# riveSunder/therldaisyworld

Hardware: AMD Instinct MI355X
Metric: cell-updates/sec (grid x batch), fused stencil+growth step (higher is better)
Workload: dtype f32

## Files before the change

### therldaisyworld_amd/csrc/dw_api.hip

```cpp
#include <hip/hip_runtime.h>

#include <cmath>
#include <cstdarg>
#include <cstdio>
#include <cstdlib>
#include <cstring>
#include <memory>
#include <new>
#include <optional>
#include <type_traits>
#include <vector>

#include "../../include/daisyworld_hip.h"
#include "dw_kernels.hpp"
#include "dw_host_util.hpp"
#include "dw_plan.hpp"
#include "dw_series.hpp"
#include "dw_episode_staging.hpp"

using namespace dw;

static thread_local char g_err[512] = "";

static int fail(int code, const char* fmt, ...) {
// ... 23 lines not shown
static thread_local int t_fail_in = 0;
struct DeviceMem {
    static int alloc(void** p, size_t n) {
        if (t_fail_in > 0 && --t_fail_in == 0) return hipErrorOutOfMemory;
        return hipMalloc(p, n);
    }
    static int release(void* p) { return hipFree(p); }
};
struct PinnedMem {
    static int alloc(void** p, size_t n) { return hipHostMalloc(p, n, hipHostMallocDefault); }
    static int release(void* p) { return hipHostFree(p); }
};
template <class T> using DevBuf = Buf<T, DeviceMem>;
template <class T> using PinnedBuf = Buf<T, PinnedMem>;

struct dw_handle {
    dw_params prm;
    hipStream_t stream = nullptr;
    bool own_stream = false;
    size_t cells = 0;
    DevBuf<plane_t> L16[2];
    DevBuf<plane_t> D16[2];
    int cur = 0;
    DevBuf<double> L64;
    DevBuf<double> D64;
    DevBuf<float> U32L;
    DevBuf<float> U32D;
    UnqKind unq_kind = UNQ_F64;
    UnqOwner unq = OWN_NONE;
    bool have_state = false;
    bool stepped = false;
    double L_last = 0.0;
    bool L_per_world = false;
    bool P_per_world = false;
    DevBuf<int> idx;
    DevBuf<double> st;
    DevBuf<int> action;
    DevBuf<int> action_tmp;
    bool have_agents = false;
    DevBuf<StatsDev> stats2[2];
    size_t stats_bytes = 0;
    int sp = 0;
    DevBuf<uint4> fixq;
    unsigned int qcap = 0;
    DevBuf<int> redo_tiles;
    Switches sw{};
// ... 82 lines not shown
        return with_bool(post, [&](auto POST) { return f(L, D, POST); });
    });
}

struct SyncOnExit {
    hipStream_t stream;
    bool armed = true;
    explicit SyncOnExit(hipStream_t s) : stream(s) {}
    ~SyncOnExit() { if (armed) (void)hipStreamSynchronize(stream); }
    void disarm() { armed = false; }
};

static int alloc_failed(int rc, const char* what, size_t bytes) {
    (void)hipGetLastError();
    const hipError_t e = static_cast<hipError_t>(rc);
    return fail(e == hipErrorOutOfMemory ? DW_ENOMEM : DW_EHIP, "allocating %s (%zu bytes) failed: %s", what, bytes,
                hipGetErrorString(e));
}
template <class B>
static int reserve(B& buf, const char* what, size_t need, size_t first_size = 0) {
    const int rc = buf.reserve(need, first_size);
    return rc ? alloc_failed(rc, what, need) : DW_OK;
}

static int alloc_group(dw_handle* h, const char* what, std::initializer_list<GroupItem<DeviceMem>> group) {
    static int fail_left = -1;
    if (h->created && fail_left < 0)
        if (const char* e = test_hook("DW_TEST_FAIL_GROUP_ALLOC")) fail_left = std::atoi(e);
    const bool armed = h->created && fail_left > 0;
    if (armed) t_fail_in = (int)group.size();
    const int rc = dw::alloc_group(group);
    if (armed && t_fail_in == 0) --fail_left;
    t_fail_in = 0;
    size_t bytes = 0;
    for (const auto& g : group) bytes += g.bytes;
    return rc ? alloc_failed(rc, what, bytes) : DW_OK;
}

static void release_unquantised(dw_handle* h) {
    if (h->unq != OWN_NONE || !h->U32L.get()) return;
    for (const auto& sn : h->snap)
        if (sn.valid && sn.unq == OWN_PREV) return;
    if (h->cells * 2 * sizeof(float) < ((size_t)1 << 30)) return;
    (void)hipStreamSynchronize(h->stream);
    h->U32L.reset();
    h->U32D.reset();
}

static void drop_unquantised_previous(dw_handle* h) {
    if (h->unq == OWN_PREV) { h->unq = OWN_NONE; h->stepped = false; }
    release_unquantised(h);
}

static int ensure_u32(dw_handle* h) {
    const size_t n = sizeof(float) * h->cells;
    return alloc_group(h, "two float32 planes", {{h->U32L, n}, {h->U32D, n}});
}

static int ensure_f64(dw_handle* h) {
    const size_t n = sizeof(double) * h->cells;
    return alloc_group(h, "two float64 planes", {{h->L64, n}, {h->D64, n}});
}

static int run_episode_impl(dw_handle* h, int32_t nsteps, const double* L_schedule, int policy_mode,
                            const uint8_t* use_table, const int8_t* table, uint32_t threshold_k,
                            uint8_t* world_alive, uint8_t* agent_ok, dw_world_stats* trace = nullptr,
                            dw_temp_stats* temps = nullptr);
static bool episode_kernel_applies(const dw_handle* h);
enum EpisodeForm { EPISODE_STEPWISE, EPISODE_WORKGROUP, EPISODE_WAVE };
static EpisodeForm episode_form(const dw_handle* h);
static EpisodeForm episode_mlp_form(const dw_handle* h, size_t* lds_bytes = nullptr);
static int worlds_per_block(int cells) { return cells <= 256 ? 4 : (cells <= 1024 ? 2 : 1); }
static int observe_into_scratch(dw_handle* h, double L_init, size_t extra_bytes, bool reward_tail = false);

static int ensure_scratch(dw_handle* h, size_t bytes) { return reserve(h->scratch, "scratch", bytes); }

static int ensure_ep_buf(dw_handle* h, size_t bytes) {
    return reserve(h->ep_buf, "the episode staging buffer", bytes, (size_t)4 << 20);
}

struct EpisodeBuffers {
    using R = EpisodeStaging;
    dw_handle* h;
    const EpisodeStaging S;
    unsigned char* img = nullptr;
    std::vector<PhysF32> p32_own;
    std::vector<unsigned char> ut_own;

    EpisodeBuffers(dw_handle* h_, const EpisodeStaging& S_) : h(h_), S(S_) {}
    bool out_direct = false;
    int alloc(bool staged, bool inputs_only = false) {
        if (int rc = ensure_ep_buf(h, S.total)) return rc;
        if (!staged) return DW_OK;
        const size_t image = inputs_only ? S.off[R::WORLD_ALIVE] : S.total;
        if (int rc = reserve(h->ep_pinned, "the page-locked episode staging", image, (size_t)1 << 20)) return rc;
        img = h->ep_pinned.get();
        out_direct = inputs_only;
        return DW_OK;
    }
    template <class T = unsigned char>
    T* dev(R::Region r) const { return S.at<T>(h->ep_buf.get(), r); }
// ... 549 lines not shown
                           o.zero_me, o.zero_n);
    } else if (exact) {
        const FusedExactArgs A = exact_args();
        with_bool(pstats != nullptr, [&](auto STATS) {
            with_fused_layout(pl, [&](auto MODE, auto PACK) {
                with_bool(pl.sym_albedo, [&](auto SYM) {
                    hipLaunchKernelGGL((step_stream_fused2_exact<MODE, PACK, STATS, SYM>), grid, dim3(256), 0, h->stream, A);
                });
            });
        });
    } else {
        with_bool(pstats != nullptr, [&](auto STATS) {
            with_fused_layout(pl, [&](auto MODE, auto PACK) {
                hipLaunchKernelGGL((step_stream_fused2<MODE, PACK, STATS>), grid, dim3(256), 0, h->stream, inL, inD, o.L, o.D, g,
                                   P1, P2, o.zero_me, o.zero_n, pstats, thr_hi);
            });
        });
    }
    HIPCHK(hipGetLastError());
    step_done(h, L2, false);
    return DW_OK;
}

static int launch_agents(dw_handle* h, const int* d_action, int act_b, int act_n, bool standalone = false,
                         double* d_reward = nullptr, unsigned char* d_done = nullptr, unsigned char* d_ok = nullptr) {
    const dw_params& p = h->prm;
    if (p.n_agents == 0) return DW_OK;
    NEED(h->have_state, DW_ESTATE, "no state uploaded");
    NEED(h->have_agents, DW_ESTATE, "no agents uploaded (call dw_upload_agents or dw_init_random)");
    NEED(p.collision_mode == 0 || standalone, DW_EINVAL,
         "collision_mode=1: call dw_update_agents, apply the collision pass (it consumes the caller's RNG) to the "
         "downloaded agent states, upload them, then dw_step without actions");
    const int blocks = (p.batch + 63) / 64;
    with_planes(h, h->unq == OWN_CUR, h->cur, [&](auto* L, auto* D) {
        using T = elem_t<decltype(L)>;
        hipLaunchKernelGGL(agents_update<T>, dim3(blocks), dim3(64), 0, h->stream, L, D, h->idx.get(), h->st.get(), d_action,
                           act_b, act_n, p.batch, p.n_agents, p.height, p.width, p.agent_gamma,
                           p.collision_mode == 0 ? 1 : 0, d_reward, d_done, d_ok);
    });
    HIPCHK(hipGetLastError());
    return DW_OK;
}

static int stage_host_actions(dw_handle* h, const int32_t* action, int b, int n) {
    const dw_params& p = h->prm;
    NEED(b >= 0 && n >= 0 && b <= p.batch && n <= p.n_agents, DW_EINVAL,
// ... 460 lines not shown
    if (!use_device_actions && nsteps >= 1 && h->have_state && !cur_quantised(h)) {
        int rc = launch_forward(h, L);
        if (rc) return rc;
        advance();
        s0 = 1;
    }
    const bool big_packed = h->plan.allow_fuse && h->plan.packed && h->cells >= ((size_t)1 << 23);
    if (!use_device_actions && nsteps - s0 > 1 && h->have_state && h->prm.height * h->prm.width <= 4096 && !big_packed &&
        (h->prm.n_agents == 0 || h->have_agents) && episode_kernel_applies(h)) {
        std::vector<double> Ls;
        while (s0 < nsteps) {
            const int k = nsteps - s0 < 4096 ? nsteps - s0 : 4096;
            Ls.resize(k);
            for (int i = 0; i < k; ++i) { Ls[i] = L; advance(); }
            int rc = run_episode_impl(h, k, Ls.data(), kPolicySkipAgents, nullptr, nullptr, 5, nullptr, nullptr);
            if (rc) return rc;
            s0 += k;
        }
        *L_io = L;
        return DW_OK;
    }
    if (!use_device_actions && h->plan.allow_fuse && h->have_state && nsteps - s0 >= 3) {
        drop_unquantised_previous(h);
        HIPCHK(hipEventRecord(h->evf0, h->stream));
        int launched = 0;
        while (nsteps - s0 >= 3) {
            const double L1 = L;
            advance();
            const double L2 = L;
            advance();
            int rc = launch_forward_fused2(h, L1, L2);
            if (rc) return rc;
            s0 += 2;
            launched += 1;
        }
        HIPCHK(hipEventRecord(h->evf1, h->stream));
        h->fused_launches = launched;
    }
    for (int s = s0; s < nsteps; ++s) {
        int rc;
        if (use_device_actions) {
            rc = launch_agents(h, h->action.get(), h->prm.batch, h->prm.n_agents);
            if (rc) return rc;
        }
        rc = launch_forward(h, L);
        if (rc) return rc;
        advance();
    }
    *L_io = L;
    return DW_OK;
}

static bool ensemble_pairs(const dw_handle* h) { return h->plan.trace_pairs && h->prm.precision == DW_PRECISION_FAST; }

static int check_per_world(const WorldRows& rows, const dw_world_params* worlds, const double* L_schedule, size_t nsteps, size_t B) {
    for (size_t i = 0; i < nsteps * B; ++i)
        NEED(std::isfinite(L_schedule[i]) && L_schedule[i] >= 0.0, DW_EINVAL,
             "L_schedule[step %zu][world %zu] = %g: a luminosity is finite and not negative", i / B, i % B, L_schedule[i]);
    for (size_t b = 0; worlds && b < B; ++b) {
        if (check_params(&rows.params(b)) != DW_OK) {
// ... 556 lines not shown
    NEED(h->have_state && h->have_agents, DW_ESTATE, "no state / agents");
    const int B = p.batch, N = p.n_agents;
    const size_t K = (size_t)nsteps, bn = (size_t)B * N;
    NEED(bn > 0, DW_EINVAL, "no agents");
    for (int b = 0; b < B; ++b) {
        NEED(!member_a || (member_a[b] >= 0 && member_a[b] < n_members), DW_EINVAL, "world %d: member out of range", b);
        NEED(!member_b || (member_b[b] >= 0 && member_b[b] < n_members), DW_EINVAL, "world %d: member out of range", b);
    }
    NEED(n_members == 1 || (member_a && member_b), DW_EINVAL, "several parameter sets need both member maps");
    NEED_SHARED_L(h, "the episode's first observation");
    const size_t wbytes = sizeof(double) * 1808 * (size_t)n_members;
    EpisodeRegions regions;
    regions.rows = K; regions.mlp = true; regions.trace = records; regions.temps = temps != nullptr;
    const EpisodeStaging S(K, (size_t)B, (size_t)N, regions);
    using R = EpisodeStaging;
    const size_t o_ma = S.off[R::MEMBER_A], o_mb = S.off[R::MEMBER_B], o_p32 = S.off[R::P32], o_ls = S.off[R::LS];
    if (temps)
        if (int rc = alloc_group(h, "the temperature reduction", {{h->temp_part, temp_part_bytes(h)}})) return rc;
    if (int erc = ensure_ep_buf(h, S.total)) return erc;
    if (params) {
        if (h->mlp_members != n_members) {
            h->mlp_w.reset();
            h->mlp_members = 0;
            if (int rc = reserve(h->mlp_w, "the parameter sets", wbytes)) return rc;
            h->mlp_members = n_members;
        }
    }
    const double* d_w = h->mlp_w.get();
    const int* d_ma = member_a ? reinterpret_cast<const int*>(h->ep_buf.get() + o_ma) : nullptr;
    const int* d_mb = member_b ? reinterpret_cast<const int*>(h->ep_buf.get() + o_mb) : nullptr;
    double* d_r = S.at<double>(h->ep_buf.get(), R::REWARD);
    unsigned char* d_d = S.at<unsigned char>(h->ep_buf.get(), R::DONE);
    StatsDev* const d_rows = S.at<StatsDev>(h->ep_buf.get(), R::TRACE);
    TempStatsDev* const d_trows = reinterpret_cast<TempStatsDev*>(h->ep_buf.get() + S.temps_off());
    SyncOnExit guard(h->stream);
    if (params) HIPCHK(hipMemcpyAsync(h->mlp_w.get(), params, wbytes, hipMemcpyHostToDevice, h->stream));
    if (member_a) HIPCHK(hipMemcpyAsync(h->ep_buf.get() + o_ma, member_a, sizeof(int) * B, hipMemcpyHostToDevice, h->stream));
    if (member_b) HIPCHK(hipMemcpyAsync(h->ep_buf.get() + o_mb, member_b, sizeof(int) * B, hipMemcpyHostToDevice, h->stream));
    const int Cc = p.height * p.width;
    const int wpb = worlds_per_block(Cc);
    size_t lds = 0;
    const EpisodeForm form = episode_mlp_form(h, &lds);
    const bool wave_kernel = form == EPISODE_WAVE, small = records ? form == EPISODE_WAVE : form != EPISODE_STEPWISE;
    if (records) lds = episode_mlp_wave_trace_lds_bytes(Cc, N);
    std::vector<PhysF32> p32;
    SyncOnExit guard2(h->stream);
    size_t t = 0;
// ... 734 lines not shown
    if (pl.kind == STEP_STREAM) {
        const StripGeom& g = pl.sgeom;
        snprintf(buf, buflen,
                 "step_stream_%s<halo=%s> wave-strip=%dx256 cells, register window + DPP neighbours, %d-row blocks in "
                 "flight%s, %d strips, grid=%d x 256 threads (4 strips each), XCD-chunked",
                 prec, halo_name[pl.halo], g.SR,
                 p.precision == DW_PRECISION_EXACT ? DW_STREAM_RB_EXACT : DW_STREAM_RB_FAST,
                 p.precision == DW_PRECISION_EXACT ? ", in-wave float64 fix-up from an LDS queue" : "", g.nstrips,
                 g.chunk * 8);
        if (pl.allow_fuse) {
            const size_t n = std::strlen(buf);
            snprintf(buf + n, buflen - n, "; dw_step_n fuses step pairs (step_stream_fused2%s%s",
                     p.precision == DW_PRECISION_EXACT ? "_exact" : "",
                     pl.seam_strips ? "_seam_pw, format buffer accesses" : (pl.fmt_planes ? "_fmt_pw, format buffer accesses" : ""));
            if (pl.seam_strips) {
                const size_t m = std::strlen(buf);
                snprintf(buf + m, buflen - m, ", seam strips: %d x %d columns + %d columns of %d row bands per wave", pl.seam_geom.ncs,
                         kSeamCols, pl.left_geom.cols_per_strip, pl.left_geom.wpr);
            }
            if (pl.row_landing) {
                const size_t m = std::strlen(buf);
                snprintf(buf + m, buflen - m, ", rows land in place: step_stream_fused2_land_seam_pw + _land_left_pw");
            }
            const size_t m = std::strlen(buf);
            snprintf(buf + m, buflen - m, ")");
        }
    } else if (pl.kind == STEP_TILED) {
        const int TR = (256 / pl.tcq) * pl.rpt;
        snprintf(buf, buflen,
                 "step_tiled<TCQ=%d,RPT=%d,%s> tile=%dx%d cells, %zu B LDS/workgroup, %d tiles, grid=%d x 256 threads, "
                 "XCD-chunked",
                 pl.tcq, pl.rpt, prec, TR, pl.tcq * 4, pl.tile_lds, pl.geom.ntiles, pl.geom.chunk * 8);
    } else {
        snprintf(buf, buflen, "step_generic<%s> one thread per cell, grid=(%d,%d) x 256 threads", prec,
                 (p.height * p.width + 255) / 256, p.batch);
    }
    {
        const size_t n = std::strlen(buf);
        snprintf(buf + n, buflen - n, pl.trace_pairs ? "; trace: step pairs" : "; trace: single steps");
    }
    {
        const size_t n = std::strlen(buf);
        snprintf(buf + n, buflen - n, pl.pw_stream ? "; per-world L: wave strips" : "; per-world L: generic");
    }
    {
        static const char* const form_name[] = {"launches per step", "workgroup (LDS)", "one wave per world"};
// ... 84 lines not shown
```

### therldaisyworld_amd/csrc/dw_plan.hpp

```cpp
#pragma once
#include <climits>
#include <cmath>
#include <cstddef>
#include <cstdio>
#include <cstdlib>
#include <cstring>

#include "../../include/daisyworld_hip.h"
#include "dw_types.hpp"

namespace dw {

struct Switches {
    bool no_sym = false, no_pack = false, no_fuse = false, no_ring = false, no_fmt_planes = false, no_seam_strips = false,
         no_row_landing = false,
         no_episode_kernel = false,
         no_episode_wave = false, no_agent_fuse = false, no_agent_preapply = false, first_f64 = false,
         first_generic = false, force_rescan = false, test_hooks = false;
    int pack_min_strips = -1, strip_rows = 0, tile_rpt = 0, queue_cap = -1, mismatch_cap = -1, trace_rows = 0, frame_ring = 0;
    double first_slack = -1.0;
    char kernel[16] = {0};
    char text[256] = {0};
};
inline const char* test_hook(const char* name) {
    return std::getenv("DW_TEST_HOOKS") ? std::getenv(name) : nullptr;
}
inline Switches read_switches() {
    Switches w;
    auto note = [&](const char* name, const char* val) {
        const size_t n = std::strlen(w.text);
        snprintf(w.text + n, sizeof(w.text) - n, "%s%s%s%s", n ? " " : "", name, val ? "=" : "", val ? val : "");
    };
    auto flag = [&](const char* name, bool& dst) { if (std::getenv(name)) { dst = true; note(name, nullptr); } };
    auto num = [&](const char* name, int& dst, bool test) {
        if (const char* e = test ? test_hook(name) : std::getenv(name)) { dst = std::atoi(e); note(name, e); }
    };
    w.test_hooks = std::getenv("DW_TEST_HOOKS") != nullptr;
    flag("DW_NO_SYM", w.no_sym); flag("DW_NO_PACK", w.no_pack); flag("DW_NO_FUSE", w.no_fuse); flag("DW_NO_RING", w.no_ring);
    flag("DW_NO_FMT_PLANES", w.no_fmt_planes); flag("DW_NO_SEAM_STRIPS", w.no_seam_strips);
    flag("DW_NO_ROW_LANDING", w.no_row_landing);
    flag("DW_NO_EPISODE_KERNEL", w.no_episode_kernel); flag("DW_NO_EPISODE_WAVE", w.no_episode_wave);
    flag("DW_NO_AGENT_FUSE", w.no_agent_fuse); flag("DW_NO_AGENT_PREAPPLY", w.no_agent_preapply);
    flag("DW_FIRST_STEP_F64", w.first_f64); flag("DW_FIRST_GENERIC", w.first_generic);
    num("DW_PACK_MIN_STRIPS", w.pack_min_strips, false); num("DW_STRIP_ROWS", w.strip_rows, false);
    num("DW_TILE_RPT", w.tile_rpt, false);
    num("DW_TEST_QUEUE_CAP", w.queue_cap, true); num("DW_TEST_MISMATCH_CAP", w.mismatch_cap, true);
    num("DW_TEST_TRACE_ROWS", w.trace_rows, true);
    num("DW_TEST_FRAME_RING", w.frame_ring, true);
    if (test_hook("DW_TEST_FORCE_RESCAN")) { w.force_rescan = true; note("DW_TEST_FORCE_RESCAN", nullptr); }
    if (const char* e = test_hook("DW_TEST_FIRST_SLACK")) { w.first_slack = std::atof(e); note("DW_TEST_FIRST_SLACK", e); }
    if (const char* e = std::getenv("DW_KERNEL")) { snprintf(w.kernel, sizeof(w.kernel), "%s", e); note("DW_KERNEL", e); }
    return w;
}

inline dw_params with_world_params(dw_params p, const dw_world_params& w) {
    p.p = w.p; p.g = w.g; p.S = w.S; p.sigma = w.sigma; p.gamma = w.gamma; p.q = w.q; p.q2 = w.q2; p.dt = w.dt;
    p.albedo_bare = w.albedo_bare; p.albedo_light = w.albedo_light; p.albedo_dark = w.albedo_dark;
    p.temp_optimal = w.temp_optimal;
    return p;
}
inline dw_world_params world_params_of(const dw_params& p) {
    return dw_world_params{p.p, p.g, p.S, p.sigma, p.gamma, p.q, p.q2, p.dt, p.albedo_bare, p.albedo_light, p.albedo_dark,
                           p.temp_optimal};
}
inline bool albedo_symmetric(double bare, double light, double dark) { return (dark - bare) == -(light - bare); }
inline bool worlds_symmetric(const dw_world_params* worlds, size_t B) {
    for (size_t b = 0; b < B; ++b)
        if (!albedo_symmetric(worlds[b].albedo_bare, worlds[b].albedo_light, worlds[b].albedo_dark)) return false;
    return true;
}

// ... 167 lines not shown
enum StepKind { STEP_GENERIC, STEP_TILED, STEP_STREAM };
struct StepPlan {
    StepKind kind = STEP_GENERIC;
    int halo = 0;
    bool packed = false;
    bool allow_fuse = false;
    int fused_mode = kFusedOvl;
    bool fmt_planes = false;
    bool seam_strips = false;
    FusedGeom seam_geom{}, left_geom{};
    bool row_landing = false;
    bool trace_pairs = false;
    bool sym_albedo = false;
    int tcq = 0, rpt = 0;
    Geom geom{};
    size_t tile_lds = 0;
    StripGeom sgeom{};
    FusedGeom fgeom{};
    int first_prec = 2;
    bool first_stream = false;
    FirstGeom first_geom{};
    bool need_fixq = false;
    bool pw_stream = false;
};

inline int halo_form(int W) { return W < 256 ? 3 : (W == 256 ? 0 : (W % 256 == 0 ? 1 : 2)); }

inline int strip_rows(long groups, int H, long target) {
    int sr = 64;
    while (sr > 8 && groups * ((H + sr - 1) / sr) < target) sr >>= 1;
    return H < sr ? H : sr;
}

inline int strip_rows_or_override(const Switches& sw, int cap, long groups, int H, long target) {
    if (sw.strip_rows < 1) return strip_rows(groups, H, target);
    const int want = sw.strip_rows < cap ? sw.strip_rows : cap;
    return H < want ? H : want;
}

inline long seam_waves_per_world(int W, int nrs) {
    const int n_full = W / kSeamCols, L = W - kSeamCols * n_full;
    const int G = L ? 64 / (L / 4 + 2) : 1;
    return (long)nrs * n_full + (L ? (nrs + G - 1) / G : 0);
}
inline bool seam_layout(const FusedGeom& f, FusedGeom* seam, FusedGeom* left) {
    const int n_full = f.W / kSeamCols, L = f.W - kSeamCols * n_full;
// ... 44 lines not shown
        if (sw.mismatch_cap >= 0 && sw.mismatch_cap < kMismatchCap) mcap = sw.mismatch_cap;
        g.force_rescan = sw.force_rescan ? 1 : 0;
        s.allow_fuse = !sw.no_fuse;
        const bool ring = p.width == 1024 && !sw.no_ring;
        s.fused_mode = p.width <= 256 ? kFusedRot : (ring ? kFusedRing : kFusedOvl);
        FusedGeom& f = s.fgeom;
        f.B = p.batch; f.H = p.height; f.W = p.width;
        f.SR = g.SR;
        f.nrs = g.nrs;
        f.lpw = g.lpw; f.wpr = g.wpr;
        f.cols_per_strip = p.width <= 256 ? 256 : (ring ? 1024 : 248);
        f.ncs = s.packed ? 1 : (p.width + f.cols_per_strip - 1) / f.cols_per_strip;
        f.nstrips = (int)(groups * f.nrs * f.ncs);
        f.nwg = ring ? f.nstrips : (f.nstrips + 3) / 4;
        f.chunk = (f.nwg + 7) / 8;
        f.qcap = g.qcap;
        f.mcap = mcap;
        f.sure_need = 9 * p.n_agents + 9 * mcap + 1;
        s.trace_pairs = s.allow_fuse && !s.packed && s.fused_mode != kFusedRing;
        s.fmt_planes = p.precision == DW_PRECISION_FAST && s.allow_fuse && !s.packed && s.fused_mode == kFusedOvl && !sw.no_fmt_planes &&
                       (size_t)p.height * p.width * sizeof(plane_t) < ((size_t)1 << 31);
        s.seam_strips = s.fmt_planes && !sw.no_seam_strips && seam_layout(f, &s.seam_geom, &s.left_geom);
        s.row_landing = s.seam_strips && !sw.no_row_landing;
    } else if (quads && p.width >= 64) {
        s.kind = STEP_TILED;
        const int Wq = p.width / 4;
        if (Wq >= 64) {
            s.tcq = 64; s.rpt = 4;
            if (sw.tile_rpt == 2 || sw.tile_rpt == 4 || sw.tile_rpt == 8) s.rpt = sw.tile_rpt;
        }
        else if (Wq >= 32) { s.tcq = 32; s.rpt = 4; }
        else { s.tcq = 16; s.rpt = 2; }
        const int TR = (256 / s.tcq) * s.rpt;
        Geom& g = s.geom;
        g.B = p.batch; g.H = p.height; g.W = p.width; g.Wq = Wq;
        g.tiles_r = (p.height + TR - 1) / TR;
        g.tiles_c = (Wq + s.tcq - 1) / s.tcq;
        g.ntiles = p.batch * g.tiles_r * g.tiles_c;
        g.chunk = (g.ntiles + 7) / 8;
        g.qcap = kMaxFix;
        if (sw.queue_cap >= 0 && sw.queue_cap < kMaxFix) g.qcap = sw.queue_cap;
        s.tile_lds = (size_t)2 * (TR + 2) * (s.tcq + 2) * 4 * sizeof(float);
    }
    s.need_fixq = p.precision == DW_PRECISION_EXACT && s.kind == STEP_TILED;
    s.pw_stream = s.kind == STEP_STREAM && !s.packed;
    s.first_prec = p.precision == DW_PRECISION_FAST ? 1 : (p.precision == DW_PRECISION_EXACT && !sw.first_f64 ? 3 : 2);
// ... 17 lines not shown
```

### therldaisyworld_amd/csrc/dw_step_fused.hpp

```cpp
#pragma once
#include <type_traits>
#include "dw_step_stream.hpp"
#include "dw_types.hpp"

namespace dw {


template <typename TI>
__device__ inline unsigned int exact1_word(const TI* __restrict__ pL, const TI* __restrict__ pD, int H, int W,
                                           int r, int c, const PhysF64& Pa) {
    const int rr = wrap_near2(r, H), cc = wrap_near2(c, W);
    const int ru = rr == 0 ? H - 1 : rr - 1, rd = rr == H - 1 ? 0 : rr + 1;
    const int cl = cc == 0 ? W - 1 : cc - 1, cr = cc == W - 1 ? 0 : cc + 1;
    const int rows[3] = {ru, rr, rd}, cols[3] = {cl, cc, cr};
    unsigned int w1[9];
#pragma unroll
    for (int x = 0; x < 3; ++x)
#pragma unroll
        for (int y = 0; y < 3; ++y) {
            const size_t o = (size_t)rows[x] * W + cols[y];
            w1[x * 3 + y] = (unsigned)(float)pL[o] | ((unsigned)(float)pD[o] << 16);
        }
    const NewCoverF64 s1 = cell_f64_lean(Pa, w1);
    return (unsigned)dw_round3_k(s1.nl) | ((unsigned)dw_round3_k(s1.nd) << 16);
// ... 10 lines not shown
            int rr = r + a - 1, cc = c + e - 1;
            rr = rr < 0 ? rr + H : (rr >= H ? rr - H : rr);
            cc = cc < 0 ? cc + W : (cc >= W ? cc - W : cc);
            const int ru = rr == 0 ? H - 1 : rr - 1, rd = rr == H - 1 ? 0 : rr + 1;
            const int cl = cc == 0 ? W - 1 : cc - 1, cr = cc == W - 1 ? 0 : cc + 1;
            const int rows[3] = {ru, rr, rd}, cols[3] = {cl, cc, cr};
            unsigned int w1[9];
#pragma unroll
            for (int x = 0; x < 3; ++x)
#pragma unroll
                for (int y = 0; y < 3; ++y) {
                    const size_t o = (size_t)rows[x] * W + cols[y];
                    w1[x * 3 + y] = (unsigned)(float)pL[o] | ((unsigned)(float)pD[o] << 16);
                }
            const NewCoverF64 s1 = cell_f64_lean(Pa, w1);
            w2[a * 3 + e] = (unsigned)dw_round3_k(s1.nl) | ((unsigned)dw_round3_k(s1.nd) << 16);
        }
    const NewCoverF64 s2 = cell_f64_lean(Pb, w2);
    kl = (float)dw_round3_k(s2.nl);
    kd = (float)dw_round3_k(s2.nd);
}

template <int MODE, bool EXACT, bool PACK = false, bool STATS = false, bool SYM = false, typename TI = plane_t,
          typename TO = plane_t, bool TRACE = false, bool FMT = false, int SEAM = kSeamNone, bool LAND = false>
__device__ __forceinline__ void fused2_body(const TI* __restrict__ inL, const TI* __restrict__ inD,
                                            TO* __restrict__ outL, TO* __restrict__ outD, const FusedGeom& G,
                                            const PhysF32& P1_, const PhysF32& P2_, const PhysF64& P64,
                                            const double& La, const double& Lb,
                                            unsigned long long* __restrict__ zero_me, int zero_n,
                                            unsigned int* __restrict__ pstats = nullptr, float thr_hi = 0.f,
                                            StatsDev* __restrict__ trace = nullptr, int trace_rescan = 0) {
    constexpr bool ROT = MODE == kFusedRot, RING = MODE == kFusedRing;
    static_assert(!RING || !PACK, "the ring exchange is written for un-packed worlds");
    static_assert(!TRACE || (!PACK && !STATS && !RING), "the trace form exists for un-packed overlapped / rotating strips");
    static_assert(SEAM == kSeamNone || FMT, "the seam strips exist for the format-access kernel");
    static_assert(!LAND || SEAM != kSeamNone, "rows land in their window slots in the two seam-strip forms");
    static_assert(!FMT || (MODE == kFusedOvl && !EXACT && !PACK && !STATS && !TRACE), "the format-access form exists for the plain float32 kernel on overlapped strips");
    __shared__ float s_edge[RING ? 2 * 4 * 8 : 1];
    __shared__ uint4 s_queue[EXACT ? 4 * kWaveQueueCap * 3 : 1];
    __shared__ unsigned int s_mm[EXACT ? 4 * kMismatchCap : 1];
    const int bid = blockIdx.x;
    const int wg = (bid & 7) * G.chunk + (bid >> 3);
    if (wg >= G.nwg) return;
    const int tid = threadIdx.x, wv = tid >> 6, lane = tid & 63;
    if (wg == 0)
        for (int i = tid; i < zero_n; i += 256) zero_me[i] = 0ull;
    const int s = RING ? wg : __builtin_amdgcn_readfirstlane(wg * 4 + wv);
    if (!RING && s >= G.nstrips) return;
    uint4* q = s_queue + (EXACT ? wv * kWaveQueueCap * 3 : 0);
    unsigned int* mm = s_mm + (EXACT ? wv * kMismatchCap : 0);
    const int spw = SEAM == kSeamLeft ? (G.nrs + G.wpr - 1) / G.wpr : G.nrs * G.ncs;
    const int b = s / spw;
    const int sw = s - b * spw;
    const int rs = SEAM == kSeamLeft ? sw * G.wpr : sw / G.ncs, cs = SEAM == kSeamLeft ? G.ncs : sw - rs * G.ncs;
    const int r0 = rs * G.SR;
    const int nr = min(G.SR, G.H - r0);
    const int band_g = SEAM == kSeamLeft ? min(lane / G.lpw, G.wpr - 1) : 0;
    const int band_j = SEAM == kSeamLeft ? min(lane - band_g * G.lpw, G.lpw - 1) : 0;
    const int band_rs = SEAM == kSeamLeft ? min(rs + band_g, G.nrs - 1) : 0;
// ... 20 lines not shown
    bool need1[4] = {true, true, true, true};
    if (PACK) { need1[0] = need1[1] = need1[2] = need1[3] = writes; }
    if (EXACT && !ROT && !RING) {
        const bool wl = __builtin_amdgcn_update_dpp(0, writes ? 1 : 0, kDppWaveShr1, 0xf, 0xf, false) != 0;
        const bool wr = __builtin_amdgcn_update_dpp(0, writes ? 1 : 0, kDppWaveShl1, 0xf, 0xf, false) != 0;
        need1[0] = writes || wl;
        need1[1] = writes;
        need1[2] = writes;
        need1[3] = writes || wr;
    }
    constexpr bool LANE_BOOLS = PACK || (STATS && MODE == kFusedOvl);
    using TieT = std::conditional_t<LANE_BOOLS, bool, unsigned long long>;
    TieT need1m[4], writes_m;
    if constexpr (LANE_BOOLS) {
        for (int i = 0; i < 4; ++i) need1m[i] = need1[i];
        writes_m = writes;
    } else {
        for (int i = 0; i < 4; ++i) need1m[i] = lane_mask(need1[i]);
        writes_m = lane_mask(writes);
    }
    const TI* pL = inL + woff;
    const TI* pD = inD + woff;

    dw_i32x4 fmt_inL, fmt_inD, fmt_outL, fmt_outD;
    int fmt_col = 0, fmt_row = 0, fmt_col_b = 0;
    if constexpr (FMT) {
        const unsigned int world_bytes = (unsigned int)(G.H * G.W) * 2u;
        fmt_inL = fmt_plane_rsrc(inL, b, world_bytes, (SEAM == kSeamStrip || LAND) ? kFmtRsrcPairs : kFmtRsrcQuads);
        fmt_inD = fmt_plane_rsrc(inD, b, world_bytes, (SEAM == kSeamStrip || LAND) ? kFmtRsrcPairs : kFmtRsrcQuads);
        fmt_outL = fmt_plane_rsrc(outL, b, world_bytes);
        fmt_outD = fmt_plane_rsrc(outD, b, world_bytes);
        fmt_col = col * 2;
        fmt_col_b = col_b * 2;
        fmt_row = G.W * 2;
    }
    struct RawIn { std::conditional_t<FMT, float4, dw_f16x4> l, d; };
    auto load_raw = [&](int rr) -> RawIn {
        RawIn w;
        if constexpr (SEAM == kSeamLeft) {
            int lr = min(rr + band_dr, r0 + band_dr + band_nr + 1);
            lr = lr < 0 ? lr + G.H : lr;
            lr = lr >= G.H ? lr - G.H : lr;
            if constexpr (LAND) {
                w.l = fmt_load2x2(fmt_inL, fmt_col + lr * fmt_row, fmt_col_b + lr * fmt_row, 0);
                w.d = fmt_load2x2(fmt_inD, fmt_col + lr * fmt_row, fmt_col_b + lr * fmt_row, 0);
                return w;
            }
            w.l = fmt_load4(fmt_inL, fmt_col + lr * fmt_row, 0);
            w.d = fmt_load4(fmt_inD, fmt_col + lr * fmt_row, 0);
            return w;
        }
        rr = min(rr, r0 + nr + 1);
        rr = rr < 0 ? rr + G.H : rr;
        rr = rr >= G.H ? rr - G.H : rr;
// ... 299 lines not shown
                up1 = up_sums4(IL[(u + 2) % 3], IL[(u + 1) % 3], ID[(u + 2) % 3], ID[(u + 1) % 3]);
                asm volatile("" : "+v"(up1.xl[0]), "+v"(up1.xl[1]), "+v"(up1.cl[0]), "+v"(up1.cl[1]),
                                  "+v"(up1.xd[0]), "+v"(up1.xd[1]), "+v"(up1.cd[0]), "+v"(up1.cd[1]));
                __builtin_amdgcn_sched_barrier(0);
                land_row(r0 + j, IL[(u + 2) % 3], ID[(u + 2) % 3]);
            }
        } else if (do1) nx = load_raw(r0 + j);
        __builtin_amdgcn_sched_barrier(0);
        float l1[4], d1[4], l2[4], d2[4];
        TieT tie1[4], tie2[4];
        float sm1 = 0.f, sm2 = 0.f;
        if (do2)
            row_cells(P2, SL[u], SL[(u + 1) % 3], SL[(u + 2) % 3], SD[u], SD[(u + 1) % 3], SD[(u + 2) % 3], l2, d2, tie2,
                      use2, st_on ? &sm2 : nullptr);
        if constexpr (LAND) {
            if constexpr (do1) cells4_up(P1, up1, IL[u], ID[u], l1, d1);
        } else if (do1)
            row_cells(P1, IL[(u + 2) % 3], IL[u], IL[(u + 1) % 3], ID[(u + 2) % 3], ID[u], ID[(u + 1) % 3], l1, d1, tie1,
                      need1m, st_on ? &sm1 : nullptr);
        if (do2) {
            row_queue(SL[u], SL[(u + 1) % 3], SL[(u + 2) % 3], SD[u], SD[(u + 1) % 3], SD[(u + 2) % 3], l2, d2, tie2, 2,
                      j - 2);
            if (st_on) stats_step2(sm2);
            if constexpr (TRACE) trace_step2(l2, d2);
            if constexpr (SEAM == kSeamLeft) {
                if (writes && j - 4 < band_nr) {
                    const int voff = fmt_col + (r0 + band_dr + j - 4) * fmt_row;
                    fmt_store4(fmt_outL, voff, 0, make_float4(l2[0], l2[1], l2[2], l2[3]));
                    fmt_store4(fmt_outD, voff, 0, make_float4(d2[0], d2[1], d2[2], d2[3]));
                }
            } else if constexpr (FMT) {
                if (writes) {
                    fmt_store4(fmt_outL, fmt_col, (r0 + j - 4) * fmt_row, make_float4(l2[0], l2[1], l2[2], l2[3]));
                    fmt_store4(fmt_outD, fmt_col, (r0 + j - 4) * fmt_row, make_float4(d2[0], d2[1], d2[2], d2[3]));
                }
            } else if (writes) {
                const size_t off = woff + (size_t)(r0 + j - 4) * G.W + col;
                stream_store4(outL + off, make_float4(l2[0], l2[1], l2[2], l2[3]));
                stream_store4(outD + off, make_float4(d2[0], d2[1], d2[2], d2[3]));
            }
        }
        if (do1) {
            row_queue(IL[(u + 2) % 3], IL[u], IL[(u + 1) % 3], ID[(u + 2) % 3], ID[u], ID[(u + 1) % 3], l1, d1, tie1, 1, j);
            if (st_on) stats_step1(sm1, l1, d1, tie1, j >= 2 && j <= nr + 1);
            if constexpr (TRACE) {
                if (decltype(MINE)::value || (j >= 2 && j <= nr + 1)) trace_step1(l1, d1, tie1);
            }
            if constexpr (RING) {
                const float4 v[4] = {make_float4(l1[0], l1[1], l1[2], l1[3]), make_float4(d1[0], d1[1], d1[2], d1[3]),
                                     widen4(nx.l), widen4(nx.d)};
                Row4* const o[4] = {&SL[u], &SD[u], &IL[(u + 2) % 3], &ID[(u + 2) % 3]};
                rows_ring(v, o, std::integral_constant<int, 4>{});
            } else if constexpr (LAND) {
                to_rows4(make_float4(l1[0], l1[1], l1[2], l1[3]), make_float4(d1[0], d1[1], d1[2], d1[3]), SL[u], SD[u]);
                __builtin_amdgcn_sched_barrier(0);
                landed(std::integral_constant<int, (SEAM == kSeamStrip && do2) ? 2 : 0>{}, IL[(u + 2) % 3], ID[(u + 2) % 3]);
                pin_edge_sums(IL[(u + 2) % 3], ID[(u + 2) % 3]);
            } else {
                to_rows4(make_float4(l1[0], l1[1], l1[2], l1[3]), make_float4(d1[0], d1[1], d1[2], d1[3]), SL[u], SD[u]);
                __builtin_amdgcn_sched_barrier(0);
                to_rows4(widen4(nx.l), widen4(nx.d), IL[(u + 2) % 3], ID[(u + 2) % 3]);
                if (!PACK) pin_edge_sums(IL[(u + 2) % 3], ID[(u + 2) % 3]);
            }
        }
    };
    using Yes = std::true_type;
    using No = std::false_type;
    iter(U1{}, Yes{}, No{}, 1, Yes{}, No{});
    iter(U2{}, Yes{}, No{}, 2, Yes{}, No{});
    iter(U0{}, Yes{}, No{}, 3, Yes{}, No{});
    const int jend = nr + 2;
    const int jloop = TRACE ? jend - 1 : jend;
    int j = 4;
    for (; j + 2 <= jloop; j += 3) {
        iter(U1{}, Yes{}, Yes{}, j, Yes{}, Yes{});
        iter(U2{}, Yes{}, Yes{}, j + 1, Yes{}, Yes{});
        iter(U0{}, Yes{}, Yes{}, j + 2, Yes{}, Yes{});
        if (EXACT && !STATS && __builtin_expect(nq >= (unsigned)flush_at, 0)) sweep_queue();
        if (CHEAP && st_sure1 && st_c2w >= (unsigned int)G.sure_need) { j += 3; break; }
    }
    if constexpr (CHEAP) {
        for (; j + 2 <= jend; j += 3) {
            iter(U1{}, Yes{}, Yes{}, j, No{}, No{});
            iter(U2{}, Yes{}, Yes{}, j + 1, No{}, No{});
            iter(U0{}, Yes{}, Yes{}, j + 2, No{}, No{});
        }
    }
    if (j <= jend) { iter(U1{}, Yes{}, Yes{}, j, Yes{}, No{}); ++j; }
    if (j <= jend) { iter(U2{}, Yes{}, Yes{}, j, Yes{}, No{}); ++j; }
    if constexpr (TRACE) {
        if (j <= jend) { iter(U0{}, Yes{}, Yes{}, j, Yes{}, No{}); ++j; }
    }
    if (j % 3 == 1) iter(U1{}, No{}, Yes{}, j, Yes{}, No{});
    else if (j % 3 == 2) iter(U2{}, No{}, Yes{}, j, Yes{}, No{});
    else iter(U0{}, No{}, Yes{}, j, Yes{}, No{});

    if (EXACT) {
        PhysF64 Pa = P64, Pb = P64;
        Pa.L = La;
        Pb.L = Lb;
        if (RING) {
            wait_row_stores_before_patching();
            __syncthreads();
        }
        sweep_queue();
        if (nmm > (unsigned)G.mcap) redo = true;
        if (RING) {
            wait_row_stores_before_patching();
            __syncthreads();
        }
        if (!redo) {
            unsigned int* s1 = reinterpret_cast<unsigned int*>(q);
            for (unsigned int m0 = 0; m0 < nmm; m0 += 2) {
// ... 139 lines not shown
                                                   __HIP_MEMORY_SCOPE_AGENT);
                    }
#pragma unroll
                    for (int jj = 0; jj < 8; ++jj) {
                        const float4 fl = widen4(__builtin_bit_cast(dw_f16x4, wl[jj])), fd = widen4(__builtin_bit_cast(dw_f16x4, wd[jj]));
                        m = fmaxf(m, fmaxf(fmaxf(fmaxf(fl.x, fl.y), fmaxf(fl.z, fl.w)), fmaxf(fmaxf(fd.x, fd.y), fmaxf(fd.z, fd.w))));
                    }
                }
                m2 = wave_max(writes ? m : 0.f);
            }
        }
        l1 = wave_sum(l1); d1 = wave_sum(d1); l2 = wave_sum(l2); d2 = wave_sum(d2);
        if (lane == 0) {
            StatsDev* const t1 = trace + b;
            StatsDev* const t2 = t1 + G.B;
            atomicMax(&t1->max_k, (unsigned int)m1);
            atomicAdd(&t1->sum_l, (unsigned long long)l1);
            atomicAdd(&t1->sum_d, (unsigned long long)d1);
            atomicMax(&t2->max_k, (unsigned int)m2);
            atomicAdd(&t2->sum_l, (unsigned long long)l2);
            atomicAdd(&t2->sum_d, (unsigned long long)d2);
        }
    }
    if (STATS) {
        if (PACK) {
            float m = st_m1;
            unsigned int c = st_c2;
            if ((G.lpw & (G.lpw - 1)) == 0) {
                for (int o = G.lpw >> 1; o > 0; o >>= 1) {
                    m = fmaxf(m, __shfl_xor(m, o, 64));
                    c += (unsigned int)__shfl_xor((int)c, o, 64);
                }
            } else {
                for (int o = 1; o < G.lpw; ++o) {
                    const int src = min(lane + o, 63);
                    m = fmaxf(m, __shfl(st_m1, src, 64));
                    c += (unsigned int)__shfl((int)st_c2, src, 64);
                }
            }
            c = c > 9u * st_nmm ? c - 9u * st_nmm : 0u;
            if (pj == 0 && writes) {
                atomicMax(&pstats[2 * (b * G.wpr + pw)], (unsigned int)m);
                if (c) atomicAdd(&pstats[2 * (b * G.wpr + pw) + 1], c);
            }
        } else {
            const float mf = wave_max(st_m1), mx = wave_max(st_x1);
// ... 138 lines not shown
```

### therldaisyworld_amd/csrc/dw_step_fused_pw.hpp

```cpp
#pragma once
#include "dw_step_fused.hpp"
#include "dw_step_per_world.hpp"

namespace dw {

__device__ __forceinline__ int pair_world(const FusedGeom& G) { return __builtin_amdgcn_readfirstlane(strip_world(G)); }

template <int MODE>
__global__ __launch_bounds__(256) __attribute__((amdgpu_waves_per_eu(DW_TRACE_FAST_WAVES, DW_TRACE_FAST_WAVES)))
void trace_pair_fast_pw(const plane_t* __restrict__ inL, const plane_t* __restrict__ inD, plane_t* __restrict__ outL,
                        plane_t* __restrict__ outD, FusedGeom G, const PairPw* __restrict__ row,
                        unsigned long long* __restrict__ zero_me, int zero_n, StatsDev* __restrict__ trace) {
    static_assert(MODE != kFusedRing, "per-world constants: a wave's strip belongs to one world");
    const PairPw& E = table_entry(row, pair_world(G));
    const PhysF64 dummy{};
    const double zero = 0.0;
    fused2_body<MODE, false, false, false, false, plane_t, plane_t, true>(inL, inD, outL, outD, G, E.P1, E.P2, dummy, zero, zero,
                                                                           zero_me, zero_n, nullptr, 0.f, trace, 0);
}

}
```

Baseline: 814.0 billion.

## Close even-length fused runs with a two-step pair kernel writing into spare planes

```diff
diff --git a/therldaisyworld_amd/csrc/dw_api.hip b/therldaisyworld_amd/csrc/dw_api.hip
--- a/therldaisyworld_amd/csrc/dw_api.hip
+++ b/therldaisyworld_amd/csrc/dw_api.hip
@@ -69,6 +69,7 @@
     DevBuf<plane_t> L16[2];
     DevBuf<plane_t> D16[2];
     int cur = 0;
+    DevBuf<plane_t> spareL, spareD;
     DevBuf<double> L64;
     DevBuf<double> D64;
     DevBuf<float> U32L;
@@ -197,6 +198,20 @@
     const int rc = buf.reserve(need, first_size);
     return rc ? alloc_failed(rc, what, need) : DW_OK;
 }
+static bool release_spare(dw_handle* h, int rc) {
+    if (rc != hipErrorOutOfMemory || !h->spareL.get()) return false;
+    (void)hipGetLastError();
+    (void)hipStreamSynchronize(h->stream);
+    h->spareL.reset();
+    h->spareD.reset();
+    return true;
+}
+template <class T>
+static int reserve(dw_handle* h, DevBuf<T>& buf, const char* what, size_t need, size_t first_size = 0) {
+    int rc = buf.reserve(need, first_size);
+    if (release_spare(h, rc)) rc = buf.reserve(need, first_size);
+    return rc ? alloc_failed(rc, what, need) : DW_OK;
+}
 
 static int alloc_group(dw_handle* h, const char* what, std::initializer_list<GroupItem<DeviceMem>> group) {
     static int fail_left = -1;
@@ -204,9 +219,11 @@
         if (const char* e = test_hook("DW_TEST_FAIL_GROUP_ALLOC")) fail_left = std::atoi(e);
     const bool armed = h->created && fail_left > 0;
     if (armed) t_fail_in = (int)group.size();
-    const int rc = dw::alloc_group(group);
-    if (armed && t_fail_in == 0) --fail_left;
+    int rc = dw::alloc_group(group);
+    const bool injected = armed && t_fail_in == 0;
+    if (injected) --fail_left;
     t_fail_in = 0;
+    if (!injected && release_spare(h, rc)) rc = dw::alloc_group(group);
     size_t bytes = 0;
     for (const auto& g : group) bytes += g.bytes;
     return rc ? alloc_failed(rc, what, bytes) : DW_OK;
@@ -225,6 +242,14 @@
 static void drop_unquantised_previous(dw_handle* h) {
     if (h->unq == OWN_PREV) { h->unq = OWN_NONE; h->stepped = false; }
     release_unquantised(h);
+}
+
+static bool ensure_spare(dw_handle* h) {
+    if (h->sw.no_spare) return false;
+    const size_t pb = sizeof(plane_t) * h->cells;
+    if (dw::alloc_group<DeviceMem>({{h->spareL, pb}, {h->spareD, pb}}) == 0) return true;
+    (void)hipGetLastError();
+    return false;
 }
 
 static int ensure_u32(dw_handle* h) {
@@ -248,10 +273,10 @@
 static int worlds_per_block(int cells) { return cells <= 256 ? 4 : (cells <= 1024 ? 2 : 1); }
 static int observe_into_scratch(dw_handle* h, double L_init, size_t extra_bytes, bool reward_tail = false);
 
-static int ensure_scratch(dw_handle* h, size_t bytes) { return reserve(h->scratch, "scratch", bytes); }
+static int ensure_scratch(dw_handle* h, size_t bytes) { return reserve(h, h->scratch, "scratch", bytes); }
 
 static int ensure_ep_buf(dw_handle* h, size_t bytes) {
-    return reserve(h->ep_buf, "the episode staging buffer", bytes, (size_t)4 << 20);
+    return reserve(h, h->ep_buf, "the episode staging buffer", bytes, (size_t)4 << 20);
 }
 
 struct EpisodeBuffers {
@@ -847,6 +872,30 @@
     return DW_OK;
 }
 
+static bool closing_pair_ready(dw_handle* h) {
+    return h->plan.closing_pair && h->plan.seam_strips && h->plan.row_landing && h->prm.precision == DW_PRECISION_FAST &&
+           ensure_spare(h);
+}
+
+static int launch_closing_pair(dw_handle* h, double L1, double L2) {
+    const StepPlan& pl = h->plan;
+    const PhysF32 P1 = derive_f32(h->prm, L1), P2 = derive_f32(h->prm, L2);
+    const StepOut o = step_out(h);
+    const FusedGeom &gs = pl.seam_geom, &gl = pl.left_geom;
+    const plane_t *inL = h->L16[h->cur].get(), *inD = h->D16[h->cur].get();
+    plane_t *midL = h->spareL.get(), *midD = h->spareD.get();
+    hipLaunchKernelGGL(close_pair_seam_pw, dim3((unsigned)gs.chunk * 8u), dim3(256), 0, h->stream, inL, inD, midL,
+                       midD, o.L, o.D, gs, P1, P2, o.stats, o.zero_me, o.zero_n);
+    if (gl.nstrips)
+        hipLaunchKernelGGL(close_pair_left_pw, dim3((unsigned)gl.chunk * 8u), dim3(256), 0, h->stream, inL, inD,
+                           midL, midD, o.L, o.D, gl, P1, P2, o.stats, o.zero_me, 0);
+    HIPCHK(hipGetLastError());
+    std::swap(h->L16[h->cur], h->spareL);
+    std::swap(h->D16[h->cur], h->spareD);
+    step_done(h, L2, true);
+    return DW_OK;
+}
+
 static int launch_agents(dw_handle* h, const int* d_action, int act_b, int act_n, bool standalone = false,
                          double* d_reward = nullptr, unsigned char* d_done = nullptr, unsigned char* d_ok = nullptr) {
     const dw_params& p = h->prm;
@@ -1353,6 +1402,7 @@
     }
     if (!use_device_actions && h->plan.allow_fuse && h->have_state && nsteps - s0 >= 3) {
         drop_unquantised_previous(h);
+        const bool closing = (nsteps - s0) % 2 == 0 && closing_pair_ready(h);
         HIPCHK(hipEventRecord(h->evf0, h->stream));
         int launched = 0;
         while (nsteps - s0 >= 3) {
@@ -1367,6 +1417,14 @@
         }
         HIPCHK(hipEventRecord(h->evf1, h->stream));
         h->fused_launches = launched;
+        if (closing && nsteps - s0 == 2) {
+            const double L1 = L;
+            advance();
+            const double L2 = L;
+            advance();
+            if (int rc = launch_closing_pair(h, L1, L2)) return rc;
+            s0 += 2;
+        }
     }
     for (int s = s0; s < nsteps; ++s) {
         int rc;
@@ -1969,7 +2027,7 @@
         if (h->mlp_members != n_members) {
             h->mlp_w.reset();
             h->mlp_members = 0;
-            if (int rc = reserve(h->mlp_w, "the parameter sets", wbytes)) return rc;
+            if (int rc = reserve(h, h->mlp_w, "the parameter sets", wbytes)) return rc;
             h->mlp_members = n_members;
         }
     }
@@ -2750,6 +2808,11 @@
                 const size_t m = std::strlen(buf);
                 snprintf(buf + m, buflen - m, ", rows land in place: step_stream_fused2_land_seam_pw + _land_left_pw");
             }
+            if (pl.closing_pair && p.precision == DW_PRECISION_FAST) {
+                const size_t m = std::strlen(buf);
+                snprintf(buf + m, buflen - m, ", even runs close on close_pair_seam_pw + close_pair_left_pw: spare planes %s",
+                         h->spareL.get() ? "held" : "not held");
+            }
             const size_t m = std::strlen(buf);
             snprintf(buf + m, buflen - m, ")");
         }
diff --git a/therldaisyworld_amd/csrc/dw_plan.hpp b/therldaisyworld_amd/csrc/dw_plan.hpp
--- a/therldaisyworld_amd/csrc/dw_plan.hpp
+++ b/therldaisyworld_amd/csrc/dw_plan.hpp
@@ -13,7 +13,7 @@
 
 struct Switches {
     bool no_sym = false, no_pack = false, no_fuse = false, no_ring = false, no_fmt_planes = false, no_seam_strips = false,
-         no_row_landing = false,
+         no_row_landing = false, no_closing_pair = false, no_spare = false,
          no_episode_kernel = false,
          no_episode_wave = false, no_agent_fuse = false, no_agent_preapply = false, first_f64 = false,
          first_generic = false, force_rescan = false, test_hooks = false;
@@ -38,7 +38,7 @@
     w.test_hooks = std::getenv("DW_TEST_HOOKS") != nullptr;
     flag("DW_NO_SYM", w.no_sym); flag("DW_NO_PACK", w.no_pack); flag("DW_NO_FUSE", w.no_fuse); flag("DW_NO_RING", w.no_ring);
     flag("DW_NO_FMT_PLANES", w.no_fmt_planes); flag("DW_NO_SEAM_STRIPS", w.no_seam_strips);
-    flag("DW_NO_ROW_LANDING", w.no_row_landing);
+    flag("DW_NO_ROW_LANDING", w.no_row_landing); flag("DW_NO_CLOSING_PAIR", w.no_closing_pair);
     flag("DW_NO_EPISODE_KERNEL", w.no_episode_kernel); flag("DW_NO_EPISODE_WAVE", w.no_episode_wave);
     flag("DW_NO_AGENT_FUSE", w.no_agent_fuse); flag("DW_NO_AGENT_PREAPPLY", w.no_agent_preapply);
     flag("DW_FIRST_STEP_F64", w.first_f64); flag("DW_FIRST_GENERIC", w.first_generic);
@@ -47,6 +47,7 @@
     num("DW_TEST_QUEUE_CAP", w.queue_cap, true); num("DW_TEST_MISMATCH_CAP", w.mismatch_cap, true);
     num("DW_TEST_TRACE_ROWS", w.trace_rows, true);
     num("DW_TEST_FRAME_RING", w.frame_ring, true);
+    if (test_hook("DW_TEST_NO_SPARE")) { w.no_spare = true; note("DW_TEST_NO_SPARE", nullptr); }
     if (test_hook("DW_TEST_FORCE_RESCAN")) { w.force_rescan = true; note("DW_TEST_FORCE_RESCAN", nullptr); }
     if (const char* e = test_hook("DW_TEST_FIRST_SLACK")) { w.first_slack = std::atof(e); note("DW_TEST_FIRST_SLACK", e); }
     if (const char* e = std::getenv("DW_KERNEL")) { snprintf(w.kernel, sizeof(w.kernel), "%s", e); note("DW_KERNEL", e); }
@@ -260,6 +261,7 @@
     FirstGeom first_geom{};
     bool need_fixq = false;
     bool pw_stream = false;
+    bool closing_pair = false;
 };
 
 inline int halo_form(int W) { return W < 256 ? 3 : (W == 256 ? 0 : (W % 256 == 0 ? 1 : 2)); }
@@ -350,6 +352,7 @@
                        (size_t)p.height * p.width * sizeof(plane_t) < ((size_t)1 << 31);
         s.seam_strips = s.fmt_planes && !sw.no_seam_strips && seam_layout(f, &s.seam_geom, &s.left_geom);
         s.row_landing = s.seam_strips && !sw.no_row_landing;
+        s.closing_pair = s.row_landing && !sw.no_closing_pair;
     } else if (quads && p.width >= 64) {
         s.kind = STEP_TILED;
         const int Wq = p.width / 4;
diff --git a/therldaisyworld_amd/csrc/dw_step_fused.hpp b/therldaisyworld_amd/csrc/dw_step_fused.hpp
--- a/therldaisyworld_amd/csrc/dw_step_fused.hpp
+++ b/therldaisyworld_amd/csrc/dw_step_fused.hpp
@@ -56,19 +56,23 @@
 }
 
 template <int MODE, bool EXACT, bool PACK = false, bool STATS = false, bool SYM = false, typename TI = plane_t,
-          typename TO = plane_t, bool TRACE = false, bool FMT = false, int SEAM = kSeamNone, bool LAND = false>
+          typename TO = plane_t, bool TRACE = false, bool FMT = false, int SEAM = kSeamNone, bool LAND = false,
+          bool CLOSE = false>
 __device__ __forceinline__ void fused2_body(const TI* __restrict__ inL, const TI* __restrict__ inD,
                                             TO* __restrict__ outL, TO* __restrict__ outD, const FusedGeom& G,
                                             const PhysF32& P1_, const PhysF32& P2_, const PhysF64& P64,
                                             const double& La, const double& Lb,
                                             unsigned long long* __restrict__ zero_me, int zero_n,
                                             unsigned int* __restrict__ pstats = nullptr, float thr_hi = 0.f,
-                                            StatsDev* __restrict__ trace = nullptr, int trace_rescan = 0) {
+                                            StatsDev* __restrict__ trace = nullptr, int trace_rescan = 0,
+                                            TO* __restrict__ midL = nullptr, TO* __restrict__ midD = nullptr,
+                                            StatsDev* __restrict__ close_stats = nullptr) {
     constexpr bool ROT = MODE == kFusedRot, RING = MODE == kFusedRing;
     static_assert(!RING || !PACK, "the ring exchange is written for un-packed worlds");
     static_assert(!TRACE || (!PACK && !STATS && !RING), "the trace form exists for un-packed overlapped / rotating strips");
     static_assert(SEAM == kSeamNone || FMT, "the seam strips exist for the format-access kernel");
     static_assert(!LAND || SEAM != kSeamNone, "rows land in their window slots in the two seam-strip forms");
+    static_assert(!CLOSE || LAND, "the closing pair is a form of the kernels whose rows land in their window slots");
     static_assert(!FMT || (MODE == kFusedOvl && !EXACT && !PACK && !STATS && !TRACE), "the format-access form exists for the plain float32 kernel on overlapped strips");
     __shared__ float s_edge[RING ? 2 * 4 * 8 : 1];
     __shared__ uint4 s_queue[EXACT ? 4 * kWaveQueueCap * 3 : 1];
@@ -135,7 +139,7 @@
     const TI* pL = inL + woff;
     const TI* pD = inD + woff;
 
-    dw_i32x4 fmt_inL, fmt_inD, fmt_outL, fmt_outD;
+    dw_i32x4 fmt_inL, fmt_inD, fmt_outL, fmt_outD, fmt_midL, fmt_midD;
     int fmt_col = 0, fmt_row = 0, fmt_col_b = 0;
     if constexpr (FMT) {
         const unsigned int world_bytes = (unsigned int)(G.H * G.W) * 2u;
@@ -143,6 +147,10 @@
         fmt_inD = fmt_plane_rsrc(inD, b, world_bytes, (SEAM == kSeamStrip || LAND) ? kFmtRsrcPairs : kFmtRsrcQuads);
         fmt_outL = fmt_plane_rsrc(outL, b, world_bytes);
         fmt_outD = fmt_plane_rsrc(outD, b, world_bytes);
+        if constexpr (CLOSE) {
+            fmt_midL = fmt_plane_rsrc(midL, b, world_bytes);
+            fmt_midD = fmt_plane_rsrc(midD, b, world_bytes);
+        }
         fmt_col = col * 2;
         fmt_col_b = col_b * 2;
         fmt_row = G.W * 2;
@@ -488,9 +496,10 @@
             row_queue(SL[u], SL[(u + 1) % 3], SL[(u + 2) % 3], SD[u], SD[(u + 1) % 3], SD[(u + 2) % 3], l2, d2, tie2, 2,
                       j - 2);
             if (st_on) stats_step2(sm2);
-            if constexpr (TRACE) trace_step2(l2, d2);
+            if constexpr (TRACE || (CLOSE && SEAM == kSeamStrip)) trace_step2(l2, d2);
             if constexpr (SEAM == kSeamLeft) {
                 if (writes && j - 4 < band_nr) {
+                    if constexpr (CLOSE) trace_step2(l2, d2);
                     const int voff = fmt_col + (r0 + band_dr + j - 4) * fmt_row;
                     fmt_store4(fmt_outL, voff, 0, make_float4(l2[0], l2[1], l2[2], l2[3]));
                     fmt_store4(fmt_outD, voff, 0, make_float4(d2[0], d2[1], d2[2], d2[3]));
@@ -518,9 +527,25 @@
                 Row4* const o[4] = {&SL[u], &SD[u], &IL[(u + 2) % 3], &ID[(u + 2) % 3]};
                 rows_ring(v, o, std::integral_constant<int, 4>{});
             } else if constexpr (LAND) {
+                constexpr bool mine = decltype(MINE)::value;
+                if constexpr (CLOSE && SEAM == kSeamLeft) {
+                    if (writes && j >= 2 && j - 2 < band_nr) {
+                        const int voff = fmt_col + (r0 + band_dr + j - 2) * fmt_row;
+                        fmt_store4(fmt_midL, voff, 0, make_float4(l1[0], l1[1], l1[2], l1[3]));
+                        fmt_store4(fmt_midD, voff, 0, make_float4(d1[0], d1[1], d1[2], d1[3]));
+                    }
+                } else if constexpr (CLOSE) {
+                    if (mine || (j >= 2 && j <= nr + 1)) {
+                        if (writes) {
+                            fmt_store4(fmt_midL, fmt_col, (r0 + j - 2) * fmt_row, make_float4(l1[0], l1[1], l1[2], l1[3]));
+                            fmt_store4(fmt_midD, fmt_col, (r0 + j - 2) * fmt_row, make_float4(d1[0], d1[1], d1[2], d1[3]));
+                        }
+                    }
+                }
                 to_rows4(make_float4(l1[0], l1[1], l1[2], l1[3]), make_float4(d1[0], d1[1], d1[2], d1[3]), SL[u], SD[u]);
                 __builtin_amdgcn_sched_barrier(0);
-                landed(std::integral_constant<int, (SEAM == kSeamStrip && do2) ? 2 : 0>{}, IL[(u + 2) % 3], ID[(u + 2) % 3]);
+                constexpr int younger = SEAM == kSeamStrip ? (do2 ? 2 : 0) + (CLOSE && mine ? 2 : 0) : 0;
+                landed(std::integral_constant<int, younger>{}, IL[(u + 2) % 3], ID[(u + 2) % 3]);
                 pin_edge_sums(IL[(u + 2) % 3], ID[(u + 2) % 3]);
             } else {
                 to_rows4(make_float4(l1[0], l1[1], l1[2], l1[3]), make_float4(d1[0], d1[1], d1[2], d1[3]), SL[u], SD[u]);
@@ -536,7 +561,7 @@
     iter(U2{}, Yes{}, No{}, 2, Yes{}, No{});
     iter(U0{}, Yes{}, No{}, 3, Yes{}, No{});
     const int jend = nr + 2;
-    const int jloop = TRACE ? jend - 1 : jend;
+    const int jloop = (TRACE || CLOSE) ? jend - 1 : jend;
     int j = 4;
     for (; j + 2 <= jloop; j += 3) {
         iter(U1{}, Yes{}, Yes{}, j, Yes{}, Yes{});
@@ -554,7 +579,7 @@
     }
     if (j <= jend) { iter(U1{}, Yes{}, Yes{}, j, Yes{}, No{}); ++j; }
     if (j <= jend) { iter(U2{}, Yes{}, Yes{}, j, Yes{}, No{}); ++j; }
-    if constexpr (TRACE) {
+    if constexpr (TRACE || CLOSE) {
         if (j <= jend) { iter(U0{}, Yes{}, Yes{}, j, Yes{}, No{}); ++j; }
     }
     if (j % 3 == 1) iter(U1{}, No{}, Yes{}, j, Yes{}, No{});
@@ -740,6 +765,17 @@
             atomicAdd(&t2->sum_d, (unsigned long long)d2);
         }
     }
+    if constexpr (CLOSE) {
+        float l2 = writes ? tr_l2.x + tr_l2.y : 0.f, d2 = writes ? tr_d2.x + tr_d2.y : 0.f;
+        const float m2 = wave_max(writes ? __int_as_float(tr_m2) : 0.f);
+        l2 = wave_sum(l2);
+        d2 = wave_sum(d2);
+        if (lane == 0) {
+            atomicMax(&close_stats[b].max_k, (unsigned int)m2);
+            atomicAdd(&close_stats[b].sum_l, (unsigned long long)l2);
+            atomicAdd(&close_stats[b].sum_d, (unsigned long long)d2);
+        }
+    }
     if (STATS) {
         if (PACK) {
             float m = st_m1;
diff --git a/therldaisyworld_amd/csrc/dw_step_fused_pw.hpp b/therldaisyworld_amd/csrc/dw_step_fused_pw.hpp
--- a/therldaisyworld_amd/csrc/dw_step_fused_pw.hpp
+++ b/therldaisyworld_amd/csrc/dw_step_fused_pw.hpp
@@ -19,4 +19,31 @@
                                                                            zero_me, zero_n, nullptr, 0.f, trace, 0);
 }
 
+#ifndef DW_CLOSE_SEAM_WAVES
+#define DW_CLOSE_SEAM_WAVES 3
+#endif
+#ifndef DW_CLOSE_LEFT_WAVES
+#define DW_CLOSE_LEFT_WAVES 3
+#endif
+__global__ __launch_bounds__(256) __attribute__((amdgpu_waves_per_eu(DW_CLOSE_SEAM_WAVES, DW_CLOSE_SEAM_WAVES)))
+void close_pair_seam_pw(const plane_t* __restrict__ inL, const plane_t* __restrict__ inD,
+                        plane_t* __restrict__ midL, plane_t* __restrict__ midD, plane_t* __restrict__ outL,
+                        plane_t* __restrict__ outD, FusedGeom G, PhysF32 P1, PhysF32 P2,
+                        StatsDev* __restrict__ stats, unsigned long long* __restrict__ zero_me, int zero_n) {
+    const PhysF64 dummy{};
+    const double zero = 0.0;
+    fused2_body<kFusedOvl, false, false, false, false, plane_t, plane_t, false, true, kSeamStrip, true, true>(
+        inL, inD, outL, outD, G, P1, P2, dummy, zero, zero, zero_me, zero_n, nullptr, 0.f, nullptr, 0, midL, midD, stats);
 }
+__global__ __launch_bounds__(256) __attribute__((amdgpu_waves_per_eu(DW_CLOSE_LEFT_WAVES, DW_CLOSE_LEFT_WAVES)))
+void close_pair_left_pw(const plane_t* __restrict__ inL, const plane_t* __restrict__ inD,
+                        plane_t* __restrict__ midL, plane_t* __restrict__ midD, plane_t* __restrict__ outL,
+                        plane_t* __restrict__ outD, FusedGeom G, PhysF32 P1, PhysF32 P2,
+                        StatsDev* __restrict__ stats, unsigned long long* __restrict__ zero_me, int zero_n) {
+    const PhysF64 dummy{};
+    const double zero = 0.0;
+    fused2_body<kFusedOvl, false, false, false, false, plane_t, plane_t, false, true, kSeamLeft, true, true>(
+        inL, inD, outL, outD, G, P1, P2, dummy, zero, zero, zero_me, zero_n, nullptr, 0.f, nullptr, 0, midL, midD, stats);
+}
+
+}
```

New measurement: 697.6 billion. 0.857x the previous value.
